# rabbitmq/ra

Measured on NVIDIA B200. Metric: committed entries/sec across N Raft groups; HBM GB/s vs roofline, higher is better.
Workload: dtype u64

## Files before the change

### ra_b200/csrc/engine.cu

```cuda
#include <cuda_runtime.h>
#include <cub/device/device_scan.cuh>
#include <cub/iterator/transform_input_iterator.cuh>
#include <stdio.h>
#include <stdlib.h>
#include <string.h>
#include <new>

#include "raft_step.cuh"
#include "raft_row.cuh"


#ifndef NST
#define NST 3
#endif
#ifndef MINB
#define MINB 5
#endif
#ifndef MINB_NARROW
#define MINB_NARROW 5
#endif
#define TILE_BYTES (RT * 64)
#define RA_BAR_WORDS 64
#define WARPS (CTA_T / 32)
#define RA_N_COUNTERS (8 + 8 * 16 + 8)
// ... 3 lines not shown
__device__ __forceinline__ void mbar_init(u64* bar, u32 count)
{ asm volatile("mbarrier.init.shared::cta.b64 [%0], %1;" :: "r"(smem_u32(bar)), "r"(count)); }
__device__ __forceinline__ void mbar_fence_init()
{ asm volatile("fence.mbarrier_init.release.cluster;" ::: "memory"); }
__device__ __forceinline__ void fence_proxy_async()
{ asm volatile("fence.proxy.async.shared::cta;" ::: "memory"); }
__device__ __forceinline__ void mbar_expect_tx(u64* bar, u32 bytes)
{ asm volatile("mbarrier.arrive.expect_tx.shared::cta.b64 _, [%0], %1;" :: "r"(smem_u32(bar)), "r"(bytes) : "memory"); }
__device__ __forceinline__ void mbar_wait(u64* bar, u32 parity)
{
#pragma unroll 1
    for (u32 spins = 0; spins < (1u << 24); spins++) {
        u32 done;
        asm volatile(
            "{\n\t.reg .pred p;\n\t"
            "mbarrier.try_wait.parity.shared::cta.b64 p, [%1], %2;\n\t"
            "selp.u32 %0, 1, 0, p;\n\t}"
            : "=r"(done) : "r"(smem_u32(bar)), "r"(parity) : "memory");
        if (done) return;
    }
    __trap();
}
__device__ __forceinline__ void tma_load_tile(void* dst_smem, const void* src_gmem, u32 bytes, u64* bar)
{
    asm volatile("cp.async.bulk.shared::cluster.global.mbarrier::complete_tx::bytes [%0], [%1], %2, [%3];"
                 :: "r"(smem_u32(dst_smem)), "l"(src_gmem), "r"(bytes), "r"(smem_u32(bar)) : "memory");
}

template <int MM, bool NARROW = false>
struct StepSmem {
    ulonglong2 stage[WARPS][NST][4 * RT];
    ulonglong2 peers_nm[PSTR * CTA_T / (NARROW ? 2 : 1)];
    u64 peers_cs[NARROW ? (PSTR > 1 ? PSTR - 1 : 1) * CTA_T / 2 : PSTR * CTA_T];
    u64 bars[WARPS][NST];
};


__device__ __forceinline__ void flush_counters(const Cols& C, u32 lane, u32 k_events, u32 k_commits, u32 k_applied,
                                               u32 k_msgs, u32 k_dropped, u32 k_elect, u32 k_fatal)
{
    if (__any_sync(0xffffffffu, (k_events | k_fatal | k_dropped | k_msgs) != 0)) {
        k_events = __reduce_add_sync(0xffffffffu, k_events); k_commits = __reduce_add_sync(0xffffffffu, k_commits);
        k_applied = __reduce_add_sync(0xffffffffu, k_applied); k_msgs = __reduce_add_sync(0xffffffffu, k_msgs);
        k_dropped = __reduce_add_sync(0xffffffffu, k_dropped); k_elect = __reduce_add_sync(0xffffffffu, k_elect);
        k_fatal = __reduce_add_sync(0xffffffffu, k_fatal);
        if (lane == 0) {
            if (k_events)  atomicAdd(&C.counters[0], (u64)k_events);
            if (k_commits) atomicAdd(&C.counters[1], (u64)k_commits);
            if (k_applied) atomicAdd(&C.counters[2], (u64)k_applied);
            if (k_msgs)    atomicAdd(&C.counters[3], (u64)k_msgs);
            if (k_dropped) atomicAdd(&C.counters[4], (u64)k_dropped);
            if (k_elect)   atomicAdd(&C.counters[5], (u64)k_elect);
            if (k_fatal)   atomicAdd(&C.counters[6], (u64)k_fatal);
        }
    }
}

template <bool SMALL> struct PlaneMask { typedef u32 type; };
template <> struct PlaneMask<false> { typedef u64 type; };
__device__ __forceinline__ u32 mask_ffs(u32 m) { return (u32)__ffs((int)m) - 1u; }
__device__ __forceinline__ u32 mask_ffs(u64 m) { return (u32)__ffsll((long long)m) - 1u; }
__device__ __forceinline__ u32 mask_or_warp(u32 m) { return __reduce_or_sync(0xffffffffu, m); }
__device__ __forceinline__ u64 mask_or_warp(u64 m)
{ return (u64)__reduce_or_sync(0xffffffffu, (u32)m) | ((u64)__reduce_or_sync(0xffffffffu, (u32)(m >> 32)) << 32); }

__device__ __forceinline__ void flush_ref_counters(const Cols& C, u32 lane, u64 c_ref)
{
    if (!__any_sync(0xffffffffu, c_ref != 0)) return;
    u32 w[4];
#pragma unroll
    for (int k = 0; k < 4; k++) {
        const u32 lo = (u32)(c_ref >> (16 * k)) & 0xffu, hi = (u32)(c_ref >> (16 * k + 8)) & 0xffu;
        w[k] = __reduce_add_sync(0xffffffffu, lo | (hi << 16));
    }
    if (lane == 0) {
#pragma unroll
        for (int k = 0; k < 4; k++) {
            if (w[k] & 0xffffu) atomicAdd(&C.counters[RA_CNT_REF + 2 * k], (u64)(w[k] & 0xffffu));
            if (2 * k + 1 < 7 && (w[k] >> 16)) atomicAdd(&C.counters[RA_CNT_REF + 2 * k + 1], (u64)(w[k] >> 16));
        }
    }
}

namespace ra_wide {
#define RA_NARROW_PASS 0
#include "raft_step_kernel.cuh"
#undef RA_NARROW_PASS
}
#ifndef RA_NO_NARROW
namespace ra_narrow {
#define RA_NARROW_PASS 1
#include "raft_step_kernel.cuh"
#undef RA_NARROW_PASS
}
#endif

__global__ void __launch_bounds__(CTA_T)
raft_general_kernel(const __grid_constant__ Cols C, const int cur, const FloodArgs F,
                    const StallCtx* __restrict__ stall_list, const u32* __restrict__ stall_count)
{
    constexpr int MM = MK_MM(0, TR_RUNTIME);
    __shared__ ulonglong2 s_peers[RA_MAX_MEMBERS * CTA_T + RA_MAX_MEMBERS * CTA_T / 2];
    const u32 tid = threadIdx.x, lane = tid & 31u;
    if (*C.abort) return;
    const u32 n = *stall_count;
    for (u32 base = blockIdx.x * CTA_T; base < n; base += gridDim.x * CTA_T) {
        const u32 i = base + tid;
        u32 k_events = 0, k_commits = 0, k_applied = 0, k_msgs = 0, k_dropped = 0, k_elect = 0, k_fatal = 0;
        u64 k_ref = 0;
        if (i < n) {
            const ulonglong2* q = reinterpret_cast<const ulonglong2*>(&stall_list[i]);
            const ulonglong2 q0 = q[0], q1 = q[1], q2 = q[2], q3 = q[3];
            const u32 r = (u32)q0.x, flags = (u32)(q0.x >> 32);
            u32 rem_mbox = (u32)q0.y, rem_loc = (u32)(q0.y >> 32);
            Member m;
            member_init(m, C, r, C.tc[r], C.lg[r], C.lw[r], C.ap[r], 0, cur, &s_peers[tid]);
            m.lrs_ok = 0;
            m.n_msgs = (u32)q1.x & 0xffffu; m.n_notes = ((u32)q1.x >> 16) & 0xffffu; m.status = (u32)(q1.x >> 32);
            m.sent_to = (u32)q1.y;
            { const u32 w = (u32)(q1.y >> 32); m.pn_type = w & 0xffu; m.pn_slot = (w >> 8) & 0xffu; m.wk = w >> 16; }
            m.pn_a = q2.x; m.pn_b = q2.y; m.pn_c = q3.x;
            u64 big = 0;
            if (flags & STALL_PENDING) {
                MT_SET(m.meta, 24, 1, 0);
                process_event<MM>(m, mk_rec(r, RA_EV_PIPELINE_RPCS, RA_NO_SLOT, 0, 0, 0, 0, 0, 0, 0, 0, 0, 0));
                m.cold &= ~8u;
            }
#pragma unroll 1
            while (rem_mbox) {
                const u32 p = __ffs(rem_mbox) - 1; rem_mbox &= rem_mbox - 1;
                const Rec e = ld_rec_plane(C.mbox[cur], C.tiles, p, r);
                big |= rec_magnitude(e);
                if (MT_FATAL(m.meta)) m.c_pack += 1u;
                else if (flood_lost<MM>(F, C, m, r, e)) m.c_pack += 1u << 20;
                else if (!note_budget_ok(m)) budget_drop_record(m);
                else if (C.pure || !fast_event<MM>(m, e)) { process_event<MM>(m, e); m.cold &= ~8u; }
            }
#pragma unroll 1
            while (rem_loc) {
                const u32 p = __ffs(rem_loc) - 1; rem_loc &= rem_loc - 1;
                const Rec e = ld_rec_plane(C.loc, C.tiles, p, r);
                big |= rec_magnitude(e);
                if (MT_FATAL(m.meta)) m.c_pack += 1u;
                else if (!note_budget_ok(m)) budget_refuse_local(m);
                else if (C.pure || !fast_event<MM>(m, e)) { process_event<MM>(m, e); m.cold &= ~8u; }
            }
            peers_writeback<MM>(m);
            k_fatal = row_end_of_step<MM>(m, C, r, cur, F);
            member_writeback(m, C, r);
            row_mark_wide(C, r, m, big);
            k_events = m.c_pack & 0xffu; k_commits = m.c_commits; k_applied = m.c_applied;
            k_msgs = (m.c_pack >> 8) & 0xffu; k_dropped = m.c_pack >> 20; k_elect = (m.c_pack >> 16) & 15u;
            k_ref = m.c_ref;
        }
        flush_counters(C, lane, k_events, k_commits, k_applied, k_msgs, k_dropped, k_elect, k_fatal);
        flush_ref_counters(C, lane, k_ref);
    }
}

__global__ void reset_empty_kernel(const Cols C)
{
    const u32 r = blockIdx.x * blockDim.x + threadIdx.x;
    if (r >= C.rows) return;
    reset_row(C, r);
}

__global__ void load_rows_kernel(const Cols C, const ra_row_state* in, u32 n)
{
    const u32 i = blockIdx.x * blockDim.x + threadIdx.x;
    if (i >= n) return;
    load_row(C, in[i]);
}

__global__ void read_rows_kernel(const Cols C, ra_row_state* out, u32 n)
{
    const u32 i = blockIdx.x * blockDim.x + threadIdx.x;
    if (i >= n) return;
    read_row(C, out[i]);
}

__global__ void load_query_kernel(const Cols C, const ra_query_state* in, u32 n)
{
    const u32 i = blockIdx.x * blockDim.x + threadIdx.x;
    if (i < n) load_query_row(C, in[i]);
}
__global__ void read_query_kernel(const Cols C, ra_query_state* out, u32 n)
// ... 451 lines not shown
    }
    if ((rc = ra_engine_reset_empty(e)) != RA_OK) goto bad;
    *out = e;
    return RA_OK;
bad:
    ra_engine_destroy(e);
    return rc;
}

template <typename T>
static int ensure(ra_engine* e, T** p, size_t* cap, size_t need)
{
    if (*cap >= need && *p) return RA_OK;
    if (*p) cudaFree(*p);
    size_t nc = need < 1024 ? 1024 : need + need / 4;
    void* q = nullptr;
    cudaError_t ce = cudaMalloc(&q, nc * sizeof(T));
    if (ce != cudaSuccess) { *p = nullptr; *cap = 0; return fail(e, ce, "cudaMalloc staging"); }
    *p = (T*)q; *cap = nc;
    return RA_OK;
}

extern "C" int ra_engine_load_rows(ra_engine* e, const ra_row_state* rows, size_t n)
{
    if (!e || (!rows && n)) return RA_E_INVAL;
    if (n == 0) return RA_OK;
    for (size_t i = 0; i < n; i++)
        if (rows[i].row >= e->C.rows || rows[i].n_members != e->C.members || !ra_row_state_valid(&rows[i])) return RA_E_INVAL;
    if (e->narrow_mode == 0 && n * 2 >= e->C.rows) {
        size_t wide = 0;
        for (size_t i = 0; i < n; i++) wide += row_state_is_wide(rows[i], e->C.members) ? 1 : 0;
        e->narrow = wide * 2 < n;
    }
    CK(cudaSetDevice(e->cfg.device));
    int rc = ensure(e, &e->d_rows, &e->d_rows_cap, n); if (rc) return rc;
    CK(cudaMemcpyAsync(e->d_rows, rows, n * sizeof(ra_row_state), cudaMemcpyHostToDevice, e->stream));
    load_rows_kernel<<<nblocks(n, 128), 128, 0, e->stream>>>(e->C, e->d_rows, (u32)n);
    CK(cudaGetLastError());
    CK(cudaStreamSynchronize(e->stream));
    return RA_OK;
}

extern "C" int ra_engine_read_rows(ra_engine* e, ra_row_state* rows, size_t n)
{
    if (!e || (!rows && n)) return RA_E_INVAL;
    if (n == 0) return RA_OK;
    for (size_t i = 0; i < n; i++) if (rows[i].row >= e->C.rows) return RA_E_INVAL;
    CK(cudaSetDevice(e->cfg.device));
    int rc = ensure(e, &e->d_rows, &e->d_rows_cap, n); if (rc) return rc;
    CK(cudaMemcpyAsync(e->d_rows, rows, n * sizeof(ra_row_state), cudaMemcpyHostToDevice, e->stream));
    read_rows_kernel<<<nblocks(n, 128), 128, 0, e->stream>>>(e->C, e->d_rows, (u32)n);
    CK(cudaGetLastError());
    CK(cudaMemcpyAsync(rows, e->d_rows, n * sizeof(ra_row_state), cudaMemcpyDeviceToHost, e->stream));
    CK(cudaStreamSynchronize(e->stream));
    return RA_OK;
}

static int query_io(ra_engine* e, ra_query_state* q, size_t n, bool load)
{
    if (!e || (!q && n)) return RA_E_INVAL;
    if (n == 0) return RA_OK;
    for (size_t i = 0; i < n; i++) if (q[i].row >= e->C.rows) return RA_E_INVAL;
    CK(cudaSetDevice(e->cfg.device));
    ra_query_state* d = nullptr;
    CK(cudaMalloc(&d, n * sizeof(ra_query_state)));
    cudaError_t ce = cudaMemcpyAsync(d, q, n * sizeof(ra_query_state), cudaMemcpyHostToDevice, e->stream);
    if (ce == cudaSuccess) {
        if (load) load_query_kernel<<<nblocks(n, 128), 128, 0, e->stream>>>(e->C, d, (u32)n);
        else {
            read_query_kernel<<<nblocks(n, 128), 128, 0, e->stream>>>(e->C, d, (u32)n);
            ce = cudaMemcpyAsync(q, d, n * sizeof(ra_query_state), cudaMemcpyDeviceToHost, e->stream);
        }
    }
    if (ce == cudaSuccess) ce = cudaGetLastError();
    if (ce == cudaSuccess) ce = cudaStreamSynchronize(e->stream);
    cudaFree(d);
    return ce == cudaSuccess ? RA_OK : fail(e, ce, "query state");
}
extern "C" int ra_engine_load_query_state(ra_engine* e, const ra_query_state* q, size_t n)
{ return query_io(e, const_cast<ra_query_state*>(q), n, true); }
extern "C" int ra_engine_read_query_state(ra_engine* e, ra_query_state* q, size_t n)
{ return query_io(e, q, n, false); }

static int launch_step(ra_engine* e, const FloodArgs& F)
{
    if (e->C.n_shards > 1) {
        if (!e->C.peer_mode) {
            if (!e->C.outbox) return RA_E_INVAL;
            cudaError_t c0 = cudaMemsetAsync(e->C.out_cnt, 0, e->C.n_shards * sizeof(u32), e->stream);
            if (c0 != cudaSuccess) return fail(e, c0, "cudaMemsetAsync out_cnt");
        }
    }
#ifdef RA_INTERLEAVE
    const u32 grid = (((e->C.tiles + WARPS - 1) / WARPS + e->C.members - 1) / e->C.members) * e->C.members;
#else
    const u32 grid = (e->C.tiles + WARPS - 1) / WARPS;
#endif
    u32* cnt = e->d_stall_cnt + (e->steps & 1), *cnt_next = e->d_stall_cnt + ((e->steps + 1) & 1);
    const int tr = !e->C.routed ? TR_HOST : (e->C.n_shards > 1 ? (e->C.peer_mode ? TR_PEER : TR_BUCKET) : TR_LOCAL);
#define LAUNCH_NS(NS, NARROW, MEMB, TRN, FLT) NS::raft_step_kernel<MK_MM(MEMB, TRN), FLT><<<grid, CTA_T, sizeof(StepSmem<MK_MM(MEMB, TRN), NARROW>), e->stream>>>( \
        e->C, e->cur, F, e->d_stall, cnt, cnt_next)
#define LAUNCH(MEMB, TRN, FLT) LAUNCH_NS(ra_wide, false, MEMB, TRN, FLT)
#ifndef RA_NO_NARROW
#define LAUNCH_N(MEMB, TRN, FLT) do { if (e->narrow) LAUNCH_NS(ra_narrow, true, MEMB, TRN, FLT); else LAUNCH_NS(ra_wide, false, MEMB, TRN, FLT); } while (0)
#else
#define LAUNCH_N(MEMB, TRN, FLT) LAUNCH_NS(ra_wide, false, MEMB, TRN, FLT)
#endif
    const bool faults = (F.drop | F.withhold | F.part) != 0;
    if (faults) {
        if (e->C.members == 5 && tr == TR_LOCAL) LAUNCH(5, TR_LOCAL, true);
        else if (e->C.members == 7 && tr == TR_LOCAL) LAUNCH(7, TR_LOCAL, true);
        else LAUNCH(0, TR_RUNTIME, true);
    } else if (e->C.members == 5) {
        switch (tr) {
        case TR_LOCAL:  LAUNCH_N(5, TR_LOCAL, false); break;
        case TR_PEER:   LAUNCH_N(5, TR_PEER, false); break;
        case TR_BUCKET: LAUNCH(5, TR_BUCKET, false); break;
        default:        LAUNCH_N(5, TR_HOST, false); break;
        }
    } else if (e->C.members == 3 && tr == TR_LOCAL) {
        LAUNCH_N(3, TR_LOCAL, false);
    } else if (e->C.members == 7 && tr == TR_LOCAL) {
        LAUNCH_N(7, TR_LOCAL, false);
    } else {
        LAUNCH(0, TR_RUNTIME, false);
    }
#undef LAUNCH
#undef LAUNCH_N
#undef LAUNCH_NS
    cudaError_t ce = cudaGetLastError();
    if (ce != cudaSuccess) return fail(e, ce, "raft_step_kernel");
    raft_general_kernel<<<e->general_grid, CTA_T, 0, e->stream>>>(e->C, e->cur, F, e->d_stall, cnt);
    ce = cudaGetLastError();
    if (ce != cudaSuccess) return fail(e, ce, "raft_general_kernel");
    if (e->C.routed) e->cur ^= 1;
    e->steps++;
    return RA_OK;
}

static bool host_ptr_mapped(const void* p, void** dev)
{
    cudaPointerAttributes a;
    if (!p || cudaPointerGetAttributes(&a, p) != cudaSuccess) { cudaGetLastError(); return false; }
    if (a.type != cudaMemoryTypeHost || !a.devicePointer) return false;
    *dev = a.devicePointer;
    return true;
}

static int enqueue_gather(ra_engine* e, IoSlot& q)
{
    int rc;
    if ((rc = ensure(e, &q.d_msgs, &q.d_msgs_cap, q.msgs_cap ? q.msgs_cap : 1))) return rc;
    if ((rc = ensure(e, &q.d_notes, &q.d_notes_cap, q.notes_cap ? q.notes_cap : 1))) return rc;
    void* dh = nullptr;
    host_ptr_mapped(q.hdr, &dh);
    const u32 R = e->C.rows;
    CK(cub::DeviceScan::ExclusiveSum(e->d_scan_tmp, e->scan_tmp_bytes, PackedIt(e->C.out_n, PackCounts()), e->d_offs,
                                     (int)(R + 1), e->stream));
    if (e->compact) {
        note_ext_count_kernel<<<nblocks((u64)R + 1, 256), 256, 0, e->stream>>>(e->C, e->d_next);
        CK(cub::DeviceScan::ExclusiveSum(e->d_scan_tmp2, e->scan_tmp2_bytes, e->d_next, e->d_xoffs, (int)(R + 1), e->stream));
        gather_out16_kernel<<<nblocks(e->C.tiles, 4), 128, 0, e->stream>>>(
            e->C, e->d_offs, e->d_xoffs, (ulonglong2*)q.d_msgs, (u64)q.msgs_cap, (ulonglong2*)q.d_notes, (u64)q.notes_cap,
            (OutHdr*)dh, e->d_err);
    } else
    gather_out_kernel<<<nblocks(e->C.tiles, 4), 128, 0, e->stream>>>(
        e->C, e->d_offs, (ulonglong2*)q.d_msgs, (u64)q.msgs_cap, (ulonglong2*)q.d_notes, (u64)q.notes_cap, (OutHdr*)dh, e->d_err);
    CK(cudaGetLastError());
    const size_t unit = e->compact ? 16 : sizeof(ra_note);
    const size_t pn = e->compact ? e->pred_notes + 2 * e->pred_ext : e->pred_notes;
    q.copied_msgs = e->pred_msgs + e->pred_msgs / 16 + (e->pred_msgs ? 16 : 0);
    q.copied_notes = pn + pn / 16 + (pn ? 64 : 0);
    if (q.copied_msgs > q.msgs_cap) q.copied_msgs = q.msgs_cap;
    if (q.copied_notes > q.notes_cap) q.copied_notes = q.notes_cap;
    if (q.copied_msgs) CK(cudaMemcpyAsync(q.user_msgs, q.d_msgs, q.copied_msgs * sizeof(ra_event), cudaMemcpyDeviceToHost, e->stream));
    if (q.copied_notes) CK(cudaMemcpyAsync(q.user_notes, q.d_notes, q.copied_notes * unit, cudaMemcpyDeviceToHost, e->stream));
    CK(cudaEventRecord(q.done, e->stream));
    return RA_OK;
}

struct EvSeg { const void* p; size_t n; };

static int submit_impl(ra_engine* e, const EvSeg* segs, size_t n_segs, bool host32,
                       ra_event* msgs, size_t msgs_cap, ra_note* notes, size_t notes_cap)
{
    if (!e || (!segs && n_segs) || (!msgs && msgs_cap) || (!notes && notes_cap)) return RA_E_INVAL;
    size_t n_ev = 0;
    for (size_t k = 0; k < n_segs; k++) { if (!segs[k].p && segs[k].n) return RA_E_INVAL; n_ev += segs[k].n; }
    if (n_ev > 0x7fffffffull) return RA_E_INVAL;
    if (e->out_pending) return RA_E_CAPACITY;
    IoSlot& q = e->io[e->io_head % RA_IO_SLOTS];
    if (e->io_head - e->io_tail >= RA_IO_SLOTS || q.busy) return RA_E_BUSY;
    CK(cudaSetDevice(e->cfg.device));
    const u32 R = e->C.rows;
    const size_t rec = host32 ? sizeof(ra_host_event) : sizeof(ra_event);
    const size_t bytes = n_ev * rec;
    if (n_ev) {
        if (q.d_ev_bytes < bytes) {
            cudaFree(q.d_ev); q.d_ev = nullptr; q.d_ev_bytes = 0;
            const size_t nb = bytes + bytes / 4 + 4096;
            CK(cudaMalloc(&q.d_ev, nb));
            q.d_ev_bytes = nb;
        }
        size_t off = 0;
        for (size_t k = 0; k < n_segs; k++) {
            if (!segs[k].n) continue;
            CK(cudaMemcpyAsync((char*)q.d_ev + off, segs[k].p, segs[k].n * rec, cudaMemcpyHostToDevice, e->copy_stream));
            off += segs[k].n * rec;
        }
        CK(cudaEventRecord(q.h2d_done, e->copy_stream));
        CK(cudaStreamWaitEvent(e->stream, q.h2d_done, 0));
    }
    if (e->loc_dirty) {
        clear_loc_kernel<<<nblocks(R, 256), 256, 0, e->stream>>>(e->C);
        e->loc_dirty = 0;
    }
// ... 109 lines not shown
                     ra_note* notes, size_t notes_cap, size_t* n_notes)
{
    if (e && e->io_head != e->io_tail) return RA_E_BUSY;
    if (!ev && n_ev) return RA_E_INVAL;
    EvSeg sg = { ev, n_ev };
    int rc = submit_impl(e, &sg, 1, host32, msgs, msgs_cap, notes, notes_cap);
    if (rc) return rc;
    return ra_engine_collect(e, n_msgs, n_notes);
}

extern "C" int ra_engine_step(ra_engine* e, const ra_event* ev, size_t n_ev,
                              ra_event* msgs, size_t msgs_cap, size_t* n_msgs,
                              ra_note*  notes, size_t notes_cap, size_t* n_notes)
{ return step_impl(e, ev, n_ev, false, msgs, msgs_cap, n_msgs, notes, notes_cap, n_notes); }

extern "C" int ra_engine_step_host(ra_engine* e, const ra_host_event* ev, size_t n_ev,
                                   ra_event* msgs, size_t msgs_cap, size_t* n_msgs,
                                   ra_note* notes, size_t notes_cap, size_t* n_notes)
{ return step_impl(e, ev, n_ev, true, msgs, msgs_cap, n_msgs, notes, notes_cap, n_notes); }

extern "C" int ra_engine_set_note_format(ra_engine* e, int compact)
{
    if (!e) return RA_E_INVAL;
    if (e->io_head != e->io_tail || e->out_pending) return RA_E_BUSY;
    CK(cudaSetDevice(e->cfg.device));
    e->compact = compact ? 1 : 0;
    e->pred_notes = e->pred_ext = 0;
    CK(cudaMemsetAsync(e->C.wc, 0, (size_t)e->C.rows * sizeof(u64), e->stream));
    CK(cudaStreamSynchronize(e->stream));
    return RA_OK;
}
extern "C" size_t ra_engine_last_ext_count(ra_engine* e) { return e ? e->last_ext : 0; }

extern "C" int ra_engine_register_host(void* p, size_t bytes)
{
    if (!p || !bytes) return RA_E_INVAL;
    return cudaHostRegister(p, bytes, cudaHostRegisterMapped | cudaHostRegisterPortable) == cudaSuccess ? RA_OK : RA_E_CUDA;
}
extern "C" int ra_engine_unregister_host(void* p)
{
    if (!p) return RA_E_INVAL;
    return cudaHostUnregister(p) == cudaSuccess ? RA_OK : RA_E_CUDA;
}

extern "C" int ra_engine_flood(ra_engine* e, uint32_t n_steps, uint32_t cmds_per_step,
                               uint32_t election_permille, uint64_t seed)
{ return ra_engine_flood_faults(e, n_steps, cmds_per_step, election_permille, seed, nullptr); }

extern "C" int ra_engine_flood_faults(ra_engine* e, uint32_t n_steps, uint32_t cmds_per_step,
                                      uint32_t election_permille, uint64_t seed, const ra_flood_faults* ff)
{
    if (!e || !e->C.routed) return RA_E_INVAL;
    if (ff && ff->partition_permille && !ff->partition_steps) return RA_E_INVAL;
    CK(cudaSetDevice(e->cfg.device));
    CK(cudaEventRecord(e->ev0, e->stream));
    for (u32 t = 0; t < n_steps; t++) {
        FloodArgs F; memset(&F, 0, sizeof F);
        F.on = 1; F.cmds = cmds_per_step; F.permille = election_permille;
        if (ff) { F.drop = ff->drop_permille; F.withhold = ff->withhold_permille; F.part = ff->partition_permille; F.part_len = ff->partition_steps; }
        F.seed = seed; F.step = e->step_no + t;
        int rc = launch_step(e, F);
        if (rc) return rc;
        if (e->flood_barrier && e->C.peer_mode) {
            e->bar_epoch++;
            peer_barrier_kernel<<<1, 32, 0, e->stream>>>(e->C, e->bar_epoch, e->d_err);
        }
    }
    CK(cudaEventRecord(e->ev1, e->stream));
    e->step_no += n_steps;
    e->loc_dirty = 1;
    e->last_launches = 2 * n_steps;
    return RA_OK;
}

extern "C" int ra_engine_stall_histogram(ra_engine* e, uint64_t* out128)
{
    if (!e || !out128) return RA_E_INVAL;
    CK(cudaSetDevice(e->cfg.device));
    CK(cudaMemcpyAsync(out128, e->C.counters + 8, 128 * sizeof(u64), cudaMemcpyDeviceToHost, e->stream));
    CK(cudaStreamSynchronize(e->stream));
    return RA_OK;
}

extern "C" int ra_engine_set_stream(ra_engine* e, void* cuda_stream)
{
    if (!e) return RA_E_INVAL;
    CK(cudaSetDevice(e->cfg.device));
    CK(cudaStreamSynchronize(e->stream));
    if (e->own_stream) cudaStreamDestroy(e->stream);
    e->stream = (cudaStream_t)cuda_stream;
    e->own_stream = 0;
    return RA_OK;
}

extern "C" int ra_engine_set_outbox(ra_engine* e, void* outbox, uint32_t* counts, uint32_t cap)
{
    if (!e || e->C.n_shards < 2 || !outbox || !counts || !cap) return RA_E_INVAL;
    e->C.outbox = (ra_event*)outbox; e->C.out_cnt = counts; e->C.out_cap = cap;
    return RA_OK;
}

extern "C" int ra_engine_deliver(ra_engine* e, const void* inbox, const uint32_t* counts, uint32_t cap)
{
    if (!e || e->C.n_shards < 2 || !inbox || !counts || !cap) return RA_E_INVAL;
    CK(cudaSetDevice(e->cfg.device));
    dim3 grid(nblocks(cap, 256) < 512 ? nblocks(cap, 256) : 512, e->C.n_shards);
    deliver_kernel<<<grid, 256, 0, e->stream>>>(e->C, e->cur, (const ra_event*)inbox, counts, cap);
    CK(cudaGetLastError());
    return RA_OK;
}

extern "C" int ra_engine_peer_get(ra_engine* e, ra_peer_ptrs* out)
{
    if (!e || !out || !e->C.routed) return RA_E_INVAL;
    for (int b = 0; b < 2; b++) { out->mbox[b] = e->C.mbox[b]; out->mbox_cnt[b] = e->C.mbox_cnt[b]; }
    return RA_OK;
}

extern "C" int ra_engine_peer_set(ra_engine* e, uint32_t shard, const ra_peer_ptrs* p)
{
    if (!e || !p || e->C.n_shards < 2 || e->C.n_shards > 8 || shard >= e->C.n_shards) return RA_E_INVAL;
    Cols& C = e->C;
    for (int b = 0; b < 2; b++) { C.peer_mbox[b][shard] = (ulonglong2*)p->mbox[b]; C.peer_cnt[b][shard] = (u64*)p->mbox_cnt[b]; }
    for (int b = 0; b < 2; b++) { C.peer_mbox[b][C.shard] = C.mbox[b]; C.peer_cnt[b][C.shard] = C.mbox_cnt[b]; }
    bool all = true;
    for (u32 k = 0; k < C.n_shards; k++) all = all && C.peer_mbox[0][k] && C.peer_mbox[1][k] && C.peer_cnt[0][k] && C.peer_cnt[1][k];
    C.peer_mode = all ? 1 : 0;
    return RA_OK;
}

extern "C" int ra_engine_peer_barrier(ra_engine* e)
{
    if (!e || !e->C.peer_mode) return RA_E_INVAL;
    CK(cudaSetDevice(e->cfg.device));
    e->bar_epoch++;
    peer_barrier_kernel<<<1, 32, 0, e->stream>>>(e->C, e->bar_epoch, e->d_err);
    CK(cudaGetLastError());
    return RA_OK;
}

extern "C" int ra_engine_set_flood_barrier(ra_engine* e, int on)
{
    if (!e) return RA_E_INVAL;
    e->flood_barrier = on ? 1 : 0;
    return RA_OK;
}

extern "C" int ra_engine_ipc_export(ra_engine* e, ra_ipc_handles* out)
{
    if (!e || !out || !e->C.routed) return RA_E_INVAL;
    CK(cudaSetDevice(e->cfg.device));
    static_assert(sizeof(cudaIpcMemHandle_t) == 64, "IPC handle size");
    CK(cudaIpcGetMemHandle((cudaIpcMemHandle_t*)out->h[0], e->C.mbox[0]));
    CK(cudaIpcGetMemHandle((cudaIpcMemHandle_t*)out->h[1], e->C.mbox[1]));
    CK(cudaIpcGetMemHandle((cudaIpcMemHandle_t*)out->h[2], e->C.mbox_cnt[0]));
    CK(cudaIpcGetMemHandle((cudaIpcMemHandle_t*)out->h[3], e->C.mbox_cnt[1]));
    return RA_OK;
}

extern "C" int ra_engine_ipc_import(ra_engine* e, uint32_t shard, const ra_ipc_handles* h)
{
    if (!e || !h) return RA_E_INVAL;
    CK(cudaSetDevice(e->cfg.device));
    ra_peer_ptrs p;
    void* q[4];
    for (int i = 0; i < 4; i++) {
// ... 56 lines not shown
```

### ra_b200/csrc/raft_logic.cuh

```cuda
#if RA_NARROW_PASS
typedef u32 ix_t;
typedef int sx_t;
#else
typedef u64 ix_t;
typedef i64 sx_t;
#endif
static constexpr ix_t IX_UNDEF = (ix_t)~(ix_t)0;
#define RA_NARROW_LIMIT 0x40000000ull
struct ixpair { ix_t x, y; };
#if RA_NARROW_PASS && defined(RA_HOST_EMU)
extern "C" void ra_emu_narrow_violation(const char* what, unsigned long long v);
__device__ __forceinline__ u64 W(ix_t v) { if (v >= 0x80000000u) ra_emu_narrow_violation("W", v); return (u64)v; }
__device__ __forceinline__ ix_t N(u64 v) { if (v >= 0x80000000ull) ra_emu_narrow_violation("N", v); return (ix_t)v; }
#else
__device__ __forceinline__ u64 W(ix_t v) { return (u64)v; }
__device__ __forceinline__ ix_t N(u64 v) { return (ix_t)v; }
#endif
#if RA_NARROW_PASS
__device__ __forceinline__ u32 lo32(ix_t v) { return v; }
__device__ __forceinline__ u32 hi32(ix_t) { return 0u; }
#else
__device__ __forceinline__ u32 lo32(ix_t v) { return (u32)(v & 0xffffffffull); }
__device__ __forceinline__ u32 hi32(ix_t v) { return (u32)(v >> 32); }
#endif
// ... 429 lines not shown
        m.lrs = idx; m.lrs_ok = 1; m.cold |= 4u;
    }
    MT_SET(m.meta, 19, 4, nr);
    m.last_idx = idx + n - 1;
    m.last_term = term;
    m.pipe_clean = 0;
    m.cold &= ~8u;
}

#if !RA_NARROW_PASS
__device__ __forceinline__ void log_truncate(Member& m, u64 idx, u64 fallback_term)
{
    u32 nr = m_nruns(m);
    m.lrs_ok = 0; m.cold = (m.cold | 4u) & ~8u;
    while (nr > 0 && run_get(m, nr - 1).x > idx) nr--;
    if (!log_nonempty(m) || idx < first_idx(m)) {
        nr = 0;
        first_idx_set(m, idx + 1);
        m.last_term = fallback_term;
    } else {
        m.last_term = run_get(m, nr - 1).y;
    }
    m.last_idx = idx;
    MT_SET(m.meta, 19, 4, nr);
}

__device__ __forceinline__ bool log_set_last_index(Member& m, u64 idx)
{
    u64 t = log_fetch_term(m, (i64)idx);
    bool has = MT_HAS_SNAP(m.meta) != 0;
    bool at_snap = has && snap_idx(m) == idx;
    if (t == RA_UNDEF && !at_snap) return false;
    if (at_snap) {
        log_truncate(m, idx, snap_term(m));
        m.last_term = snap_term(m);
        m.lw_idx = snap_idx(m); m.lw_term = snap_term(m);
        return true;
    }
    u64 lwidx = idx < m.lw_idx ? idx : m.lw_idx;
    u64 lwterm = (has && snap_idx(m) == lwidx) ? snap_term(m) : log_fetch_term(m, (i64)lwidx);
    log_truncate(m, idx, t);
    m.last_term = t;
    m.lw_idx = lwidx; m.lw_term = lwterm;
    return true;
}

__device__ __forceinline__ void log_handle_written(Member& m, u64 term, u64 from, u64 to)
{
    u64 cur = to;
    bool has = MT_HAS_SNAP(m.meta) != 0;
    for (int guard = 0; guard < 2 * RA_MAX_RUNS + 4; guard++) {
        bool in = log_nonempty(m) && cur >= first_idx(m) && cur <= m.last_idx;
        if (in) {
            u64 s, t, e; run_find(m, cur, s, t, e);
            if (t == term) { m.lw_idx = cur; m.lw_term = term; return; }
            u64 lo = s > first_idx(m) ? s : first_idx(m);
            if (from > lo) return;
            if (lo == 0 || lo - 1 < from) return;
            cur = lo - 1;
            continue;
        }
        if (has && cur <= snap_idx(m)) return;
        if (cur > m.last_idx) {
            u64 stop = cur < snap_idx(m) ? cur : snap_idx(m);
            if (has && snap_idx(m) > m.last_idx && stop >= from) return;
            if (m.last_idx < from) return;
            cur = m.last_idx;
            if (!(log_nonempty(m))) return;
            continue;
        }
        return;
    }
}

#endif


__device__ __forceinline__ void set_fatal(Member& m, u32 code)
{
    if (!(m.status & RA_ST_FATAL)) m.status |= RA_ST_FATAL | ((code & 0xffu) << 20);
    MT_SET(m.meta, 26, 1, 1);
}

__device__ __noinline__ void note_store_raw(ra_note* slot_ptr, u32 row, u32 type, u32 slot, u32 aux, u64 a, u64 b, u64 c)
{
    ulonglong2* q = reinterpret_cast<ulonglong2*>(slot_ptr);
    q[0] = make_ulonglong2((u64)row | ((u64)(type & 0xff) << 32) | ((u64)(slot & 0xff) << 40) | ((u64)(aux & 0xffff) << 48), a);
    q[1] = make_ulonglong2(b, c);
}
__device__ __forceinline__ void note_store(Member& m, u32 k, u32 type, u32 slot, u32 aux, u64 a, u64 b, u64 c)
{
    note_store_raw(&m.C->onote[(size_t)k * m.C->rows + m.row], m.row, type, slot, aux, a, b, c);
}

__device__ __noinline__ void put_local(ulonglong2* loc, u32 tiles, u32 k, u32 row, u32 type, u32 n, u64 term, u64 a, u64 b)
{
    ulonglong2* q = loc + rec_word(tiles, k, row, 0);
    q[0] = make_ulonglong2((u64)type | ((u64)RA_NO_SLOT << 8) | ((u64)RS_PLAIN << 24) | ((u64)(n & 0xffff) << 32), term);
    q[RT] = make_ulonglong2(a, b);
}

__device__ __forceinline__ void note_flush(Member& m, u32 aux = 0)
{
    if (m.pn_type == RA_NOTE_NONE) return;
    note_store(m, m.n_notes - 1, m.pn_type, m.pn_slot, aux, W(m.pn_a), W(m.pn_b), W(m.pn_c));
    if (m.pn_type == RA_NOTE_WAL_APPEND) {
        const u32 n = m.wk & 3u;
        m.wk = (n < 2 ? n + 1 : 2u) | ((m.n_notes - 1) << 4) | ((m.wk & 0xf0u) << 4);
    }
    m.pn_type = RA_NOTE_NONE;
}

__device__ __forceinline__ void note(Member& m, u32 type, u32 slot, ix_t a, ix_t b, ix_t c)
{
    if (m.pn_type == type && type == RA_NOTE_WAL_APPEND && m.pn_c == c && m.pn_b + 1 == a) { m.pn_b = b; return; }
    if (m.pn_type == type && type == RA_NOTE_APPLY && m.pn_b + 1 == a) { m.pn_b = b; return; }
    if (m.n_notes >= m.C->note_cap - 1) {
        m.status |= RA_ST_NOTE_OVERFLOW; set_fatal(m, RA_FATAL_NOTE_OVERFLOW); return;
    }
    note_flush(m);
    m.n_notes++;
    m.pn_type = type; m.pn_slot = slot; m.pn_a = a; m.pn_b = b; m.pn_c = c;
}

#ifdef RA_NO_BUDGET
__device__ __forceinline__ bool note_budget_ok(const Member&) { return true; }
#else
__device__ __forceinline__ bool note_budget_ok(const Member& m) { return m.n_notes + RA_NOTE_RESERVE + 1u <= m.C->note_cap; }
#endif
__device__ __forceinline__ void budget_drop_record(Member& m)
{ m.status |= RA_ST_NOTE_OVERFLOW | RA_ST_MSG_DROPPED; m.c_pack += 1u << 20; }
__device__ __forceinline__ void budget_refuse_local(Member& m)
{ m.status |= RA_ST_NOTE_OVERFLOW; m.status += 1u << 28; }

template <int MM>
__device__ __forceinline__ void emit_msg(Member& m, u32 to, Rec r)
{
    const Cols& C = *m.C;
    u32 dst = to * C.groups + m.group;
    const bool is_next = (R_flags(r) & RA_EVF_NEXT_EVENT) != 0;
    const bool routed = MTR == TR_RUNTIME ? (C.routed != 0) : (MTR != TR_HOST);
    if (routed && !is_next && to >= NMEM(C)) return;
    if (!is_next) R_set_from(r, m.slot);
    R_clear_pad(r);
    if (routed && !is_next) {
        u32 k = (m.sent_to >> (4 * to)) & 7u;
        if (k >= RA_MBOX_DEPTH) { m.status |= RA_ST_MSG_DROPPED; m.c_pack += 1u << 20; return; }
        R_set_row_seq(r, dst, k);
        const bool sharded = MTR == TR_RUNTIME ? (C.n_shards > 1) : (MTR == TR_PEER || MTR == TR_BUCKET);
        if (sharded) {
            const u32 ds = (C.shard + to + 8u * C.n_shards - m.slot) % C.n_shards;
            const bool peer = MTR == TR_RUNTIME ? (C.peer_mode != 0) : (MTR == TR_PEER);
            if (peer) {
                if (st_rec_plane(C.peer_mbox[m.nb][ds], C.tiles, m.slot * RA_MBOX_DEPTH + k, dst, r)) m.sent_to |= 8u << (4 * to);
                m.sent_to += 1u << (4 * to);
                m.c_pack += 1u << 8;
                return;
            }
            if (ds != C.shard) {
                const u32 act = __activemask();
                const u32 grp = __match_any_sync(act, ds);
                const u32 ldr = __ffs(grp) - 1;
                u32 base = 0;
                if ((threadIdx.x & 31u) == ldr) base = atomicAdd(&C.out_cnt[ds], (u32)__popc(grp));
                base = __shfl_sync(grp, base, ldr);
                const u32 pos = base + __popc(grp & ((1u << (threadIdx.x & 31u)) - 1u));
                if (pos >= C.out_cap) { m.status |= RA_ST_MSG_DROPPED; m.c_pack += 1u << 20; return; }
                st_rec(&C.outbox[(size_t)ds * C.out_cap + pos], r);
                m.sent_to += 1u << (4 * to);
                m.c_pack += 1u << 8;
                return;
            }
        }
        if (st_rec_plane(C.mbox[m.nb], C.tiles, m.slot * RA_MBOX_DEPTH + k, dst, r)) m.sent_to |= 8u << (4 * to);
        m.sent_to += 1u << (4 * to);
        m.c_pack += 1u << 8;
        return;
    }
// ... 1032 lines not shown
```

### ra_b200/csrc/raft_step_kernel.cuh

```cuda
#if RA_NARROW_PASS
#define RA_STEP_MINB MINB_NARROW
#else
#define RA_STEP_MINB MINB
#endif
template <int MM, bool FAULTS>
__global__ void __launch_bounds__(CTA_T, RA_STEP_MINB)
raft_step_kernel(const __grid_constant__ Cols C, const int cur, const FloodArgs F,
                 StallCtx* __restrict__ stall_list, u32* __restrict__ stall_count, u32* __restrict__ stall_count_next)
{
    extern __shared__ __align__(128) unsigned char smem_raw[];
    typedef StepSmem<MM, RA_NARROW_PASS != 0> Smem;
    Smem& S = *reinterpret_cast<Smem*>(smem_raw);
    const u32 tid = threadIdx.x, lane = tid & 31u, warp = tid >> 5;
#ifdef RA_INTERLEAVE
    u32 wtile;
    {
        const u32 k = C.members, per = gridDim.x / k;
        wtile = ((blockIdx.x % k) * per + blockIdx.x / k) * WARPS + warp;
    }
#else
    const u32 wtile = blockIdx.x * WARPS + warp;
#endif
    const u32 r = wtile * RT + lane;
    const bool valid = r < C.rows;
    u32 k_events = 0, k_commits = 0, k_applied = 0, k_msgs = 0, k_dropped = 0, k_elect = 0, k_fatal = 0;
    u64 k_ref = 0;
    if (blockIdx.x == 0 && tid == 0) *stall_count_next = 0;

    const ulonglong2 z2 = make_ulonglong2(0, 0);
    ulonglong2 ap = z2, tc = z2, lg = z2, lw = z2;
    u64 cntw = 0, lrs = 0; u32 nloc = 0;
#if RA_NARROW_PASS
    u32 wfb = 0;
#endif
    if (valid) {
        ap = C.ap[r];
        nloc = C.loc_n[r];
#if RA_NARROW_PASS
        wfb = C.wf[r];
#endif
        if (C.routed) cntw = C.mbox_cnt[cur][r];
        tc = C.tc[r]; lg = C.lg[r]; lw = C.lw[r]; lrs = C.lrs[r];
    }
    if (*C.abort) return;
    const bool fatal0 = MT_FATAL(ap.y) != 0;
    const bool pending = valid && MT_PIPE_PEND(ap.y) != 0;
    constexpr u32 NPM = (MMEM ? MMEM : RA_MAX_MEMBERS) * RA_MBOX_DEPTH;
    typedef typename PlaneMask<(NPM + RA_LOCAL_CAP <= 32)>::type mask_t;
    mask_t mine = 0;
    u32 my_tail = 0;
    if (valid && !fatal0) {
        u32 mb = 0;
        for (u32 s = 0; s < NMEM(C); s++) {
            const u32 c = (u32)(cntw >> (8 * s)) & 0xffu;
            mb |= ((1u << (c & 7u)) - 1u) << (RA_MBOX_DEPTH * s);
            my_tail |= ((c >> 3) & 1u) << s;
        }
        mine = (mask_t)mb | ((mask_t)((1u << (nloc & 7u)) - 1u) << NPM);
        my_tail |= nloc & 0xff00u;
    }
    const bool work = valid && (F.on || nloc || cntw || pending);
    mask_t todo = mask_or_warp(mine);
    const u32 w_tail = __reduce_or_sync(0xffffffffu, my_tail);
    if (!__any_sync(0xffffffffu, work)) return;
    u64* bars = &S.bars[warp][0];
    if (lane == 0) {
        for (int i = 0; i < NST; i++) mbar_init(&bars[i], 1);
        mbar_fence_init();
    }
    __syncwarp();

    Member m;
#if RA_NARROW_PASS
    member_init(m, C, valid ? r : 0, tc, lg, lw, ap, lrs, cur, reinterpret_cast<ulonglong2*>(reinterpret_cast<uint2*>(S.peers_nm) + tid));
#else
    member_init(m, C, valid ? r : 0, tc, lg, lw, ap, lrs, cur, &S.peers_nm[tid]);
#endif
    m.row = r;
#if RA_NARROW_PASS
    const bool wide_row = wfb != 0;
#else
    const bool wide_row = false;
#endif
    if (work && !fatal0 && !wide_row && MT_ROLE(ap.y) == RA_LEADER) peers_prefetch<MM>(m);

    bool stalled = false;
    u32 stall_flags = 0;

    mask_t rem = 0;
    if (work && ((!fatal0 && pending) || wide_row)) {
        stalled = true; stall_flags = (!fatal0 && pending) ? STALL_PENDING : 0u; rem = mine;
    }
    mask_t toissue = todo;
    u32 n_issued = 0, n_done = 0, st_issue = 0, st = 0, par = 0;
#pragma unroll 1
    while (todo) {
        if (lane == 0) {
#pragma unroll 1
            while (toissue && n_issued < n_done + NST) {
                const u32 q = mask_ffs(toissue); toissue &= toissue - 1;
                const size_t plane_words = (size_t)C.tiles * (4 * RT);
                const ulonglong2* src = (q < NPM ? C.mbox[cur] + (size_t)q * plane_words
                                                 : C.loc + (size_t)(q - NPM) * plane_words) + (size_t)wtile * (4 * RT);
                const u32 tbit = q < NPM ? q / RA_MBOX_DEPTH : 8u + q - NPM;
                const u32 bytes = ((w_tail >> tbit) & 1u) ? TILE_BYTES : TILE_BYTES / 2;
                fence_proxy_async();
                mbar_expect_tx(&bars[st_issue], bytes);
                tma_load_tile(&S.stage[warp][st_issue][0], src, bytes, &bars[st_issue]);
                n_issued++; st_issue = st_issue + 1 == NST ? 0 : st_issue + 1;
            }
        }
        const u32 p = mask_ffs(todo); todo &= todo - 1;
        const bool my = !stalled && ((mine >> p) & 1u);
        mbar_wait(&bars[st], par);
        if (my) {
            const ulonglong2* sp = &S.stage[warp][st][0];
            const ulonglong2 c0 = sp[lane], c1 = sp[RT + lane];
            ulonglong2 t2 = make_ulonglong2(0, 0), t3 = t2;
            if (rec_has_tail(c0)) { t2 = sp[2 * RT + lane]; t3 = sp[3 * RT + lane]; }
            Rec e;
            const bool fits = rec_decode(c0, c1, t2, t3, r, e);
            if (MT_FATAL(m.meta)) m.c_pack += 1u;
            else if (FAULTS && p < NPM && flood_lost<MM>(F, C, m, r, e)) m.c_pack += 1u << 20;
            else if (!fits || !note_budget_ok(m) || C.pure || !fast_event<MM>(m, e)) {
                stalled = true;
                rem = mine & ~(((mask_t)1 << p) - 1);
                atomicAdd(&C.counters[8 + (m_role(m) & 7u) * 16 + (R_type(e) & 15u)], 1ull);
            }
        }
        n_done++;
        if (++st == NST) { st = 0; par ^= 1u; }
        __syncwarp();
    }
    const u32 rem_mbox = (u32)(rem & (((mask_t)1 << (NPM - 1) << 1) - 1)), rem_loc = (u32)(rem >> (NPM - 1) >> 1);

    if (work) {
        if (cntw && !fatal0) C.mbox_cnt[cur][r] = 0;
        if (nloc) C.loc_n[r] = 0;
        if ((m.pstate & 3u) == 2u) asm volatile("cp.async.wait_all;" ::: "memory");
        peers_writeback<MM>(m);
        if (!stalled) k_fatal = row_end_of_step<MM, FAULTS>(m, C, r, cur, F);
        if (!wide_row) member_writeback(m, C, r);
        k_events = m.c_pack & 0xffu; k_commits = m.c_commits; k_applied = m.c_applied;
        k_msgs = (m.c_pack >> 8) & 0xffu; k_dropped = m.c_pack >> 20; k_elect = (m.c_pack >> 16) & 15u;
        k_ref = m.c_ref;
    }
    const u32 sm = __ballot_sync(0xffffffffu, stalled);
    if (sm) {
        u32 base = 0;
        if (lane == 0) base = atomicAdd(stall_count, (u32)__popc(sm));
        base = __shfl_sync(0xffffffffu, base, 0);
        if (stalled) {
            ulonglong2* q = reinterpret_cast<ulonglong2*>(&stall_list[base + __popc(sm & ((1u << lane) - 1u))]);
            q[0] = make_ulonglong2((u64)r | ((u64)stall_flags << 32), (u64)rem_mbox | ((u64)rem_loc << 32));
            q[1] = make_ulonglong2((u64)(m.n_msgs | (m.n_notes << 16)) | ((u64)m.status << 32),
                                   (u64)m.sent_to | ((u64)(m.pn_type | (m.pn_slot << 8) | (m.wk << 16)) << 32));
            q[2] = make_ulonglong2(W(m.pn_a), W(m.pn_b));
            q[3] = make_ulonglong2(W(m.pn_c), 0);
        }
    }
    flush_counters(C, lane, k_events, k_commits, k_applied, k_msgs, k_dropped, k_elect, k_fatal);
    flush_ref_counters(C, lane, k_ref);
}

#undef RA_STEP_MINB
```

Baseline: 1.237 billion.

## Chain step kernels with programmatic dependent launch and inline note stores

Launches the step and general kernels with programmatic stream serialization, and each kernel calls griddepcontrol.wait followed immediately by launch_dependents. This lets the next kernel's launch and prologue overlap the tail of the previous one, cutting inter-kernel launch gaps across the many per-step launches. It also turns two noinline store helpers into forceinline, which removes call overhead but may raise register pressure. An optional compile-time per-warp timeline probe is added but is off by default.

```diff
diff --git a/ra_b200/csrc/engine.cu b/ra_b200/csrc/engine.cu
--- a/ra_b200/csrc/engine.cu
+++ b/ra_b200/csrc/engine.cu
@@ -109,6 +109,23 @@
     }
 }
 
+__device__ __forceinline__ void grid_dep_wait() { asm volatile("griddepcontrol.wait;" ::: "memory"); }
+__device__ __forceinline__ void grid_dep_launch() { asm volatile("griddepcontrol.launch_dependents;" ::: "memory"); }
+
+#ifdef RA_WARP_TIMELINE
+struct WarpTimeline {
+    u64 t_entry, t_inputs, t_loop, t_exit;
+    u32 tile;
+    u32 info;
+    u32 pad[2];
+};
+#define RA_WTL_CAP (1u << 16)
+__device__ WarpTimeline g_wtl[RA_WTL_CAP];
+__device__ __forceinline__ u64 wtl_now(u32 dep)
+{ u64 t; asm volatile("mov.u64 %0, %%globaltimer;" : "=l"(t) : "r"(dep) : "memory"); return t; }
+__device__ __forceinline__ u32 wtl_smid() { u32 s; asm volatile("mov.u32 %0, %%smid;" : "=r"(s)); return s; }
+#endif
+
 namespace ra_wide {
 #define RA_NARROW_PASS 0
 #include "raft_step_kernel.cuh"
@@ -129,6 +146,8 @@
     constexpr int MM = MK_MM(0, TR_RUNTIME);
     __shared__ ulonglong2 s_peers[RA_MAX_MEMBERS * CTA_T + RA_MAX_MEMBERS * CTA_T / 2];
     const u32 tid = threadIdx.x, lane = tid & 31u;
+    grid_dep_wait();
+    grid_dep_launch();
     if (*C.abort) return;
     const u32 n = *stall_count;
     for (u32 base = blockIdx.x * CTA_T; base < n; base += gridDim.x * CTA_T) {
@@ -746,6 +765,18 @@
 extern "C" int ra_engine_read_query_state(ra_engine* e, ra_query_state* q, size_t n)
 { return query_io(e, q, n, false); }
 
+template <typename... P, typename... A>
+static cudaError_t launch_chained(void (*k)(P...), u32 grid, size_t smem, cudaStream_t s, A... a)
+{
+    cudaLaunchConfig_t cfg = {};
+    cfg.gridDim = dim3(grid); cfg.blockDim = dim3(CTA_T); cfg.dynamicSmemBytes = smem; cfg.stream = s;
+    cudaLaunchAttribute at[1];
+    at[0].id = cudaLaunchAttributeProgrammaticStreamSerialization;
+    at[0].val.programmaticStreamSerializationAllowed = 1;
+    cfg.attrs = at; cfg.numAttrs = 1;
+    return cudaLaunchKernelEx(&cfg, k, a...);
+}
+
 static int launch_step(ra_engine* e, const FloodArgs& F)
 {
     if (e->C.n_shards > 1) {
@@ -762,8 +793,9 @@
 #endif
     u32* cnt = e->d_stall_cnt + (e->steps & 1), *cnt_next = e->d_stall_cnt + ((e->steps + 1) & 1);
     const int tr = !e->C.routed ? TR_HOST : (e->C.n_shards > 1 ? (e->C.peer_mode ? TR_PEER : TR_BUCKET) : TR_LOCAL);
-#define LAUNCH_NS(NS, NARROW, MEMB, TRN, FLT) NS::raft_step_kernel<MK_MM(MEMB, TRN), FLT><<<grid, CTA_T, sizeof(StepSmem<MK_MM(MEMB, TRN), NARROW>), e->stream>>>( \
-        e->C, e->cur, F, e->d_stall, cnt, cnt_next)
+    cudaError_t ce = cudaSuccess;
+#define LAUNCH_NS(NS, NARROW, MEMB, TRN, FLT) ce = launch_chained(NS::raft_step_kernel<MK_MM(MEMB, TRN), FLT>, grid, \
+        sizeof(StepSmem<MK_MM(MEMB, TRN), NARROW>), e->stream, e->C, e->cur, F, e->d_stall, cnt, cnt_next)
 #define LAUNCH(MEMB, TRN, FLT) LAUNCH_NS(ra_wide, false, MEMB, TRN, FLT)
 #ifndef RA_NO_NARROW
 #define LAUNCH_N(MEMB, TRN, FLT) do { if (e->narrow) LAUNCH_NS(ra_narrow, true, MEMB, TRN, FLT); else LAUNCH_NS(ra_wide, false, MEMB, TRN, FLT); } while (0)
@@ -792,10 +824,11 @@
 #undef LAUNCH
 #undef LAUNCH_N
 #undef LAUNCH_NS
-    cudaError_t ce = cudaGetLastError();
+    if (ce == cudaSuccess) ce = cudaGetLastError();
     if (ce != cudaSuccess) return fail(e, ce, "raft_step_kernel");
-    raft_general_kernel<<<e->general_grid, CTA_T, 0, e->stream>>>(e->C, e->cur, F, e->d_stall, cnt);
-    ce = cudaGetLastError();
+    ce = launch_chained(raft_general_kernel, e->general_grid, 0, e->stream, e->C, e->cur, F,
+                        (const StallCtx*)e->d_stall, (const u32*)cnt);
+    if (ce == cudaSuccess) ce = cudaGetLastError();
     if (ce != cudaSuccess) return fail(e, ce, "raft_general_kernel");
     if (e->C.routed) e->cur ^= 1;
     e->steps++;
@@ -1071,6 +1104,26 @@
     return RA_OK;
 }
 
+#ifdef RA_WARP_TIMELINE
+extern "C" int ra_debug_warp_timeline(ra_engine* e, void* out, size_t cap, size_t* n, int clear)
+{
+    if (!e || !n) return RA_E_INVAL;
+    CK(cudaSetDevice(e->cfg.device));
+    CK(cudaStreamSynchronize(e->stream));
+    size_t k = e->C.tiles < RA_WTL_CAP ? e->C.tiles : RA_WTL_CAP;
+    if (k > cap) k = cap;
+    if (out && k) CK(cudaMemcpyFromSymbol(out, g_wtl, k * sizeof(WarpTimeline)));
+    if (clear) {
+        void* p = nullptr;
+        CK(cudaGetSymbolAddress(&p, g_wtl));
+        CK(cudaMemset(p, 0, sizeof(WarpTimeline) * RA_WTL_CAP));
+    }
+    CK(cudaDeviceSynchronize());
+    *n = k;
+    return RA_OK;
+}
+#endif
+
 extern "C" int ra_engine_set_stream(ra_engine* e, void* cuda_stream)
 {
     if (!e) return RA_E_INVAL;
diff --git a/ra_b200/csrc/raft_logic.cuh b/ra_b200/csrc/raft_logic.cuh
--- a/ra_b200/csrc/raft_logic.cuh
+++ b/ra_b200/csrc/raft_logic.cuh
@@ -535,7 +535,7 @@
     MT_SET(m.meta, 26, 1, 1);
 }
 
-__device__ __noinline__ void note_store_raw(ra_note* slot_ptr, u32 row, u32 type, u32 slot, u32 aux, u64 a, u64 b, u64 c)
+__device__ __forceinline__ void note_store_raw(ra_note* slot_ptr, u32 row, u32 type, u32 slot, u32 aux, u64 a, u64 b, u64 c)
 {
     ulonglong2* q = reinterpret_cast<ulonglong2*>(slot_ptr);
     q[0] = make_ulonglong2((u64)row | ((u64)(type & 0xff) << 32) | ((u64)(slot & 0xff) << 40) | ((u64)(aux & 0xffff) << 48), a);
@@ -546,7 +546,7 @@
     note_store_raw(&m.C->onote[(size_t)k * m.C->rows + m.row], m.row, type, slot, aux, a, b, c);
 }
 
-__device__ __noinline__ void put_local(ulonglong2* loc, u32 tiles, u32 k, u32 row, u32 type, u32 n, u64 term, u64 a, u64 b)
+__device__ __forceinline__ void put_local(ulonglong2* loc, u32 tiles, u32 k, u32 row, u32 type, u32 n, u64 term, u64 a, u64 b)
 {
     ulonglong2* q = loc + rec_word(tiles, k, row, 0);
     q[0] = make_ulonglong2((u64)type | ((u64)RA_NO_SLOT << 8) | ((u64)RS_PLAIN << 24) | ((u64)(n & 0xffff) << 32), term);
diff --git a/ra_b200/csrc/raft_step_kernel.cuh b/ra_b200/csrc/raft_step_kernel.cuh
--- a/ra_b200/csrc/raft_step_kernel.cuh
+++ b/ra_b200/csrc/raft_step_kernel.cuh
@@ -8,6 +8,8 @@
 raft_step_kernel(const __grid_constant__ Cols C, const int cur, const FloodArgs F,
                  StallCtx* __restrict__ stall_list, u32* __restrict__ stall_count, u32* __restrict__ stall_count_next)
 {
+    grid_dep_wait();
+    grid_dep_launch();
     extern __shared__ __align__(128) unsigned char smem_raw[];
     typedef StepSmem<MM, RA_NARROW_PASS != 0> Smem;
     Smem& S = *reinterpret_cast<Smem*>(smem_raw);
@@ -22,6 +24,9 @@
     const u32 wtile = blockIdx.x * WARPS + warp;
 #endif
     const u32 r = wtile * RT + lane;
+#ifdef RA_WARP_TIMELINE
+    const u64 wtl_t0 = wtl_now(r);
+#endif
     const bool valid = r < C.rows;
     u32 k_events = 0, k_commits = 0, k_applied = 0, k_msgs = 0, k_dropped = 0, k_elect = 0, k_fatal = 0;
     u64 k_ref = 0;
@@ -63,6 +68,10 @@
     mask_t todo = mask_or_warp(mine);
     const u32 w_tail = __reduce_or_sync(0xffffffffu, my_tail);
     if (!__any_sync(0xffffffffu, work)) return;
+#ifdef RA_WARP_TIMELINE
+    const u64 wtl_t1 = wtl_now(w_tail ^ (u32)ap.y);
+    const bool wtl_leaders = __all_sync(0xffffffffu, valid && MT_ROLE(ap.y) == RA_LEADER);
+#endif
     u64* bars = &S.bars[warp][0];
     if (lane == 0) {
         for (int i = 0; i < NST; i++) mbar_init(&bars[i], 1);
@@ -132,6 +141,9 @@
         if (++st == NST) { st = 0; par ^= 1u; }
         __syncwarp();
     }
+#ifdef RA_WARP_TIMELINE
+    const u64 wtl_t2 = wtl_now(n_done);
+#endif
     const u32 rem_mbox = (u32)(rem & (((mask_t)1 << (NPM - 1) << 1) - 1)), rem_loc = (u32)(rem >> (NPM - 1) >> 1);
 
     if (work) {
@@ -161,6 +173,14 @@
     }
     flush_counters(C, lane, k_events, k_commits, k_applied, k_msgs, k_dropped, k_elect, k_fatal);
     flush_ref_counters(C, lane, k_ref);
+#ifdef RA_WARP_TIMELINE
+    const u64 wtl_t3 = wtl_now(lane);
+    if (lane == 0 && wtile < RA_WTL_CAP) {
+        WarpTimeline& w = g_wtl[wtile];
+        w.t_entry = wtl_t0; w.t_inputs = wtl_t1; w.t_loop = wtl_t2; w.t_exit = wtl_t3;
+        w.tile = wtile; w.info = (wtl_smid() & 0xffffu) | ((wtl_leaders ? 1u : 0u) << 16) | ((n_done & 0xffu) << 24);
+    }
+#endif
 }
 
 #undef RA_STEP_MINB
```

Measured after the change: 1.332 billion (median of 6 runs). 7.7% higher.
